# ckawoalt/Deep-Q-Learning_TRON

Hardware: AMD Instinct MI355X
Metric: env-steps/sec (higher is better)
Workload: dtype i8; 1 GPU; 65536 parallel 24x24 TRON envs per GPU, mode=none, random actions (in-kernel Philox), autoreset, obs=codes for both players; synthetic persistent rollout (no consumer reads the intermediate observations); envs_per_gpu=65536, grid=24x24, parallelism=env-shard x1

## Files before the change

### deep-q-learning_tron_amd/csrc/tron_env.hip

```cpp
#include "tron_device.hpp"
#include "tron_minimax.hpp"
#include "../../include/tron_hip.h"

#include <hip/hip_runtime.h>
#include <stdint.h>
#include <stdio.h>
#include <stdlib.h>
#include <math.h>
#include <string.h>
#include <new>
#include <type_traits>
#include <type_traits>

using namespace tron;

namespace {

constexpr int WAVE = 64;
constexpr int BLOCK = 256;
constexpr int DK = 6;

struct StepOut {
    int8_t *done;
    int8_t *winner;
// ... 801 lines not shown
    tally = 0u;
}

template <bool TAPE>
__device__ __forceinline__ void roll_helper(const Params &P, int env, bool autoreset, const uint4 &st, const uint4 &rs, int k_steps,
                                            int lane, uint2 *aring, uint32_t *sring, const uint32_t *cring, const StepOut &out,
                                            int wave, int gw, bool mine, const int8_t *tape, uint32_t game_starts, uint32_t *hand, bool handed)
{
    ROLL_HSTAMP(0);
    const uint32_t seed = P.seed, stream = P.stream;
    const int W = P.W, fair = P.fair, S = P.S;
    const uint32_t tick0 = st.w - ((autoreset && (st.y & META_DONE)) ? 1u : 0u), ep0 = rs.y;
    const int nb = (k_steps + ROLL_R - 1) / ROLL_R;
    uint32_t *abytes = reinterpret_cast<uint32_t *>(aring);
    uint32_t hi = 0u;
    uint32_t *const hme = hand + (mine ? (size_t)env : 0u);
    const size_t hn = (size_t)P.N;
    bool have_actions = false;
    if (handed) {
        uint32_t hw[ROLL_HAND_DWORDS];
#pragma unroll
        for (int i = 0; i < ROLL_HAND_DWORDS; ++i) hw[i] = 0u;
        hw[ROLL_HAND_DWORDS - 1] = ep0 + 2u * (uint32_t)ROLL_R;
        if (mine) {
            const uint32_t *q = hme;
#pragma unroll
            for (int i = 0; i < ROLL_HAND_DWORDS; ++i, q += hn) hw[i] = *q;
        }
#pragma unroll
        for (int i = 0; i < 2 * ROLL_R; ++i) sring[i * WAVE + lane] = hw[i];
        hi = hw[ROLL_HAND_DWORDS - 1] - ep0;
        if constexpr (!TAPE) {
            have_actions = __all(hw[2 * ROLL_R + 1] != ROLL_HAND_NO_ACTIONS) != 0;
            if (have_actions) aring[lane] = make_uint2(hw[2 * ROLL_R], hw[2 * ROLL_R + 1]);
        }
    }
    for (int b = -1; b < nb; ++b) {
        uint32_t base = 0u;
        if (b > 0) {
            ROLL_HSTAMP_BLOCK(b, 0);
            __syncthreads();
            ROLL_HSTAMP_BLOCK(b, 1);
        }
        const bool last = b + 1 >= nb;
        if (last && !autoreset) break;
        if (b >= 0) base = (b ? cring[(b & 1) * WAVE + lane] : 0u) + (uint32_t)ROLL_R;
        const uint32_t to = base + (uint32_t)min(ROLL_R, k_steps - (last ? b : b + 1) * ROLL_R);
        if (last) {
            if constexpr (!TAPE) {
#pragma nounroll
                for (int d = 0; d < ROLL_R / 4; ++d) {
                    uint32_t v = 0u;
#pragma unroll
                    for (uint32_t i = 0; i < 4u; ++i) {
                        uint32_t x[4];
                        philox4x32_10((uint32_t)env, tick0 + (uint32_t)k_steps + (uint32_t)(d * 4) + i, RNG_STEP, 0u, seed, stream, x);
                        v |= action_byte(x[0], x[1]) << (8u * i);
                    }
                    if (mine) hme[(size_t)(2 * ROLL_R + d) * hn] = v;
                }
            } else if (mine) {
                hme[(size_t)(2 * ROLL_R + 1) * hn] = ROLL_HAND_NO_ACTIONS;
            }
        } else if (TAPE || !(b < 0 && have_actions)) {
            if constexpr (!TAPE) {
#pragma nounroll
                for (int d = 0; d < ROLL_R / 4; ++d) {
                    const uint32_t s0 = (uint32_t)((b + 1) * ROLL_R + d * 4);
                    uint32_t v = 0u;
#pragma unroll
                    for (uint32_t i = 0; i < 4u; ++i) {
                        uint32_t x[4];
                        philox4x32_10((uint32_t)env, tick0 + s0 + i, RNG_STEP, 0u, seed, stream, x);
                        v |= action_byte(x[0], x[1]) << (8u * i);
                    }
                    abytes[(((s0 / ROLL_R) & 1u) * WAVE + (uint32_t)lane) * (ROLL_R / 4) + ((s0 / 4u) & (ROLL_R / 4 - 1))] = v;
                }
            } else {
                const int s0 = (b + 1) * ROLL_R;
                const uint16_t *row = reinterpret_cast<const uint16_t *>(tape) + (size_t)s0 * (size_t)P.N + (size_t)env;
                uint32_t t[ROLL_R];
#pragma unroll
                for (int i = 0; i < ROLL_R; ++i) t[i] = (mine && s0 + i < k_steps) ? row[(size_t)i * (size_t)P.N] : 0u;
                uint32_t v[2] = {0u, 0u};
#pragma unroll
                for (int i = 0; i < ROLL_R; ++i) v[i >> 2] |= ((t[i] & 3u) | ((t[i] >> 6) & 0xCu)) << (8 * (i & 3));
                aring[((b + 1) & 1) * WAVE + lane] = make_uint2(v[0], v[1]);
            }
        }
        if (autoreset) {
            const uint32_t upto = b < 0 ? to - min(game_starts, to) : to;
#pragma nounroll
            for (uint32_t j = hi + 1u; j <= upto; ++j)
                sring[((ep0 + j) & (2u * ROLL_R - 1u)) * WAVE + (uint32_t)lane] = start_cells_word(S, make_game_starts(seed, stream, W, fair, (uint32_t)env, ep0 + j));
            hi = max(hi, to);
        }
        if (last) {
            if (mine) {
                uint32_t hw[2 * ROLL_R];
#pragma unroll
                for (int i = 0; i < 2 * ROLL_R; ++i) hw[i] = sring[i * WAVE + lane];
                uint32_t *q = hme;
#pragma unroll
                for (int i = 0; i < 2 * ROLL_R; ++i, q += hn) *q = hw[i];
                q[2u * hn] = ep0 + hi;
            }
            ROLL_HSTAMP(ROLL_HSTAMPS - 2);
            break;
        }
        if (b < 0) {
            ROLL_HSTAMP(1);
            ROLL_HSTAMP(2);
            __syncthreads();
            ROLL_HSTAMP(3);
        }
    }
}

__device__ __forceinline__ int roll_cell(int S, int r, int c) { return __mul24(r + 1, S) + (c + 1); }
typedef __attribute__((address_space(3))) uint32_t lds_u32;
__device__ __forceinline__ uint32_t lds_cell_dword(uint32_t board_lds, uint32_t cell) { return board_lds + (cell >> 3) * 4u; }
__device__ __forceinline__ uint32_t lds_cell_shift(uint32_t cell) { return (cell & 7u) * 4u; }
__device__ __forceinline__ void lds_set_nibble(uint32_t dword_lds, uint32_t shift, uint32_t nib)
{
    asm volatile("ds_mskor_b32 %0, %1, %2" : : "v"(dword_lds), "v"(0xFu << shift), "v"(nib << shift) : "memory");
}

template <bool TAPE, bool REC = false>
__device__ __forceinline__ void roll_resident(kernarg_t *kp, int E, int epw, uint32_t cpe, uint32_t flags, const StepOut &out,
                                              int k_steps, unsigned char *smem, const int8_t *tape, unsigned long long *emask, uint32_t *hand)
{
    const uint32_t sd = 2u * cpe + 1u;
    uint32_t *boards = reinterpret_cast<uint32_t *>(smem);
    uint32_t *tmpl = boards + (size_t)E * sd;

    const int tid = threadIdx.x;
    const int lane = tid & 63;
    const int gw = (int)(blockDim.x >> 7);
    const int hw_wave = __builtin_amdgcn_readfirstlane(tid >> 6);
    const bool helper = hw_wave >= gw;
    const int wave = helper ? hw_wave - gw : hw_wave;
    uint16_t *wlist = reinterpret_cast<uint16_t *>(tmpl + 2u * cpe + (size_t)wave * (32u * cpe));
    uint32_t *rings = tmpl + ((2u * cpe + (size_t)gw * (32u * cpe) + 1u) & ~(size_t)1u) + (size_t)wave * ROLL_RING_DWORDS;
    uint2 *aring = reinterpret_cast<uint2 *>(rings);
    uint32_t *sring = rings + 4 * WAVE;
    uint32_t *cring = sring + 2 * ROLL_R * WAVE;
    const bool autoreset = (flags & TRON_STEP_AUTORESET) != 0u, nonrev = !TAPE && (flags & TRON_STEP_NONREVERSING) != 0u;
    const int we0 = wave * epw;
    const int e0 = (int)blockIdx.x * E + we0;
    const int env = e0 + lane;
    uint32_t *wboards = boards + (size_t)we0 * sd;
    uint32_t *board = wboards + (size_t)lane * sd;
    unsigned char *cellb = reinterpret_cast<unsigned char *>(board);
    bool mine;
    int8_t *oenv;
    uint4 st = make_uint4(0u, 0u, 0u, 0u), rs = make_uint4(0u, 0u, 0u, 0u);
    uint2 ab = make_uint2(0u, 0u);
    unsigned long long mask = 0ull;
    unsigned long long dirty = 0ull;
    unsigned long long stale = 0ull;
    bool st_dirty = false;
    uint32_t nres = 0u;
    uint32_t n_steps = 0u, n_w1 = 0u, n_w2 = 0u, n_draw = 0u;
    uint32_t tally = 0u;
    int S = 0;

    ROLL_STAMP_LAUNCH(0);
    {
        Params P;
        load_params_scalar(P, kp);
        const int G = P.G;
        S = P.S;
        const int ne = min(min(epw, E - we0), P.N - e0);
        mine = lane < ne;
        oenv = P.obs_state + (size_t)(mine ? env : 0) * 2u * G;
        const bool masked = (flags & ROLL_ENTRY_MASKED) != 0u;
        const bool handed = (flags & ROLL_ENTRY_HANDED) != 0u;
        const uint32_t game_starts = masked && autoreset && !handed ? (uint32_t)min(ROLL_GAME_STARTS, min(ROLL_R, k_steps)) : 0u;
        if (mine) {
            st = P.st4[env];
            if (autoreset) rs = P.rs4[env];
            if (masked && !helper) mask = emask[env];
        }
        for (uint32_t d = (uint32_t)tid; d < 2u * cpe; d += blockDim.x) {
            const uint32_t *fw = reinterpret_cast<const uint32_t *>(P.fresh);
            const uint32_t last = (uint32_t)G / 4u - 1u;
            const uint32_t f[2] = {fw[min(2u * d, last)], fw[min(2u * d + 1u, last)]};
            uint32_t v = 0u;
#pragma unroll
            for (uint32_t j = 0; j < 8u; ++j)
                if (d * 8u + j < (uint32_t)G)
                    v |= ((int8_t)(f[j >> 2] >> (8u * (j & 3u))) == TRON_EMPTY ? NIB_EMPTY : NIB_WALL) << (4u * j);
            tmpl[d] = v;
        }
        __syncthreads();
        if (helper) {
            roll_helper<TAPE>(P, env, autoreset, st, rs, k_steps, lane, aring, sring, cring, out, wave, gw, mine, tape, game_starts, hand, handed);
            return;
        }
        if (masked) {
            stale = ~mask & (cpe >= 64u ? ~0ull : (1ull << cpe) - 1ull);
            unsigned long long m = mask;
            const uint32_t cnt = (uint32_t)__popcll(m);
            uint32_t pos = 0u, T = 0u;
#pragma unroll
            for (uint32_t b = 0; b < 7u; ++b) {
                const unsigned long long bm = __ballot(((cnt >> b) & 1u) != 0u);
                pos += __builtin_amdgcn_mbcnt_hi((uint32_t)(bm >> 32), __builtin_amdgcn_mbcnt_lo((uint32_t)bm, 0u)) << b;
                T += (uint32_t)__popcll(bm) << b;
            }
            if (T) {
                for (uint32_t p = pos; m; ++p) {
                    wlist[p] = (uint16_t)(((uint32_t)lane << 6) | ((uint32_t)__ffsll((long long)m) - 1u));
                    m &= m - 1ull;
                }
                __builtin_amdgcn_fence(__ATOMIC_ACQ_REL, "wavefront");
                __builtin_amdgcn_wave_barrier();
                const int8_t *const obase = P.obs_state + (size_t)e0 * 2u * G;
                constexpr uint32_t GF = 8u;
                for (uint32_t t0 = 0u; t0 < T; t0 += 64u * GF) {
                    uint32_t ent[GF];
                    uint4 v[GF];
#pragma unroll
                    for (uint32_t j = 0; j < GF; ++j) ent[j] = wlist[min(t0 + 64u * j + (uint32_t)lane, T - 1u)];
#pragma unroll
                    for (uint32_t j = 0; j < GF; ++j)
                        if (t0 + 64u * j < T)
                            v[j] = load_chunk<true>(obase + (__umul24(ent[j] >> 6, 2u * (uint32_t)G) + (ent[j] & 63u) * 16u));
#pragma unroll
                    for (uint32_t j = 0; j < GF; ++j)
                        if (t0 + 64u * j < T && t0 + 64u * j + (uint32_t)lane < T) {
                            const uint32_t own = ent[j] >> 6, k = ent[j] & 63u;
                            const int nb = G - (int)k * 16;
                            if (nb <= 4) v[j].y = 0u;
                            if (nb <= 8) v[j].z = 0u;
                            if (nb <= 12) v[j].w = 0u;
                            uint32_t *b = wboards + __umul24(own, sd) + 2u * k;
                            b[0] = pack_codes8(v[j].x, v[j].y);
                            b[1] = pack_codes8(v[j].z, v[j].w);
                        }
                }
                __builtin_amdgcn_fence(__ATOMIC_ACQ_REL, "wavefront");
                __builtin_amdgcn_wave_barrier();
            }
            if (game_starts) {
                const uint32_t to = (uint32_t)min(ROLL_R, k_steps);
#pragma nounroll
                for (uint32_t j = to - game_starts + 1u; j <= to; ++j)
                    sring[((rs.y + j) & (2u * ROLL_R - 1u)) * WAVE + (uint32_t)lane] = start_cells_word(S, make_game_starts(P.seed, P.stream, P.W, P.fair, (uint32_t)env, rs.y + j));
            }
        } else {
            const bool ck = (uint32_t)lane < cpe;
            const int nb = G - lane * 16;
            const uint32_t t0 = ck ? tmpl[2 * lane] : 0u, t1 = ck ? tmpl[2 * lane + 1] : 0u;
            constexpr int PF = 8;
            for (int e = 0; e < ne; e += PF) {
                uint4 v[PF];
#pragma unroll
                for (int j = 0; j < PF; ++j)
                    v[j] = load_chunk<true>(P.obs_state + (size_t)(e0 + min(e + j, ne - 1)) * 2u * G + (ck ? lane * 16 : 0));
#pragma unroll
                for (int j = 0; j < PF; ++j) {
                    if (e + j >= ne) break;
                    uint32_t p0 = 0u, p1 = 0u;
                    if (ck) {
                        if (nb <= 4) v[j].y = 0u;
                        if (nb <= 8) v[j].z = 0u;
                        if (nb <= 12) v[j].w = 0u;
                        p0 = pack_codes8(v[j].x, v[j].y);
                        p1 = pack_codes8(v[j].z, v[j].w);
                        uint32_t *b = wboards + (size_t)(e + j) * sd + 2 * lane;
                        b[0] = p0;
                        b[1] = p1;
                    }
                    const unsigned long long diff = __ballot(ck && (p0 != t0 || p1 != t1));
                    if (lane == e + j) mask = diff;
                }
            }
        }
        ROLL_HSTAMP(ROLL_HSTAMPS - 1);
        __syncthreads();
    }
    const unsigned long long mask0 = mask;
    size_t row = 0;

    int cell[2];
    {
        int r[2], c[2];
        unpack_pos(st.x, r, c);
        cell[0] = roll_cell(S, r[0], c[0]);
        cell[1] = roll_cell(S, r[1], c[1]);
    }
    const uint32_t deltas = cell_deltas(S);
    uint32_t alive = st.y & 3u;
    bool done = (st.y & META_DONE) != 0u;
    int winner = (int)((st.y >> 4) & 3u);
    uint32_t last[2] = {(st.y >> 8) & 0xFu, (st.y >> 12) & 0xFu};
    if (mine && !done) dirty = (1ull << (cell[0] >> 4)) | (1ull << (cell[1] >> 4));
    uint32_t eplen = st.z, tick = st.w;
    rs.z = start_cells_word(S, rs.z);
    const uint32_t board_lds = (uint32_t)(uintptr_t)(lds_u32 *)board;
    uint32_t hdw[2] = {lds_cell_dword(board_lds, (uint32_t)cell[0]), lds_cell_dword(board_lds, (uint32_t)cell[1])};
    uint32_t hsh[2] = {lds_cell_shift((uint32_t)cell[0]), lds_cell_shift((uint32_t)cell[1])};

    for (int s0 = 0; s0 < k_steps; s0 += ROLL_R) {
        if (s0) {
            if (out.totals && (s0 & 127) == 0) roll_flush_tally(tally, n_steps, n_w1, n_w2, n_draw);
            cring[((s0 / ROLL_R) & 1) * WAVE + lane] = nres;
            __syncthreads();
        }
        ab = aring[((s0 / ROLL_R) & 1) * WAVE + lane];
        asm volatile("" : "+v"(ab.x), "+v"(ab.y));
        const int s1 = min(s0 + ROLL_R, k_steps);
        auto block_steps = [&](auto nr) __attribute__((always_inline)) {
        constexpr bool NONREV = decltype(nr)::value;
#pragma nounroll
        for (int s = s0; s < s1; ++s) {
            Params P;
            if constexpr (REC) load_params_scalar(P, kp);
            ROLL_STAMP(0);

            const bool stepped = mine && !done;
            float rw0 = 0.0f, rw1 = 0.0f;
            if (stepped) {
                const uint32_t abyte = ab.x & 0xFFu;
                const int a[2] = {draw_action_byte(abyte, 0, last[0], NONREV), draw_action_byte(abyte, 1, last[1], NONREV)};
                int ncell[2];
                unsigned long long nbit[2];
                uint32_t nk[2], ndw[2], nsh[2];
#pragma unroll
                for (int p = 0; p < 2; ++p) {
                    ncell[p] = cell[p] + cell_delta(deltas, a[p]);
                    nk[p] = (uint32_t)ncell[p] >> 4;
                    asm("" : "+v"(nk[p]));
                    nbit[p] = 1ull << nk[p];
                    ndw[p] = lds_cell_dword(board_lds, (uint32_t)ncell[p]);
                    nsh[p] = lds_cell_shift((uint32_t)ncell[p]);
                }
                uint32_t bw[2], tc0[2], tc1[2];
                bool sl[2];
#pragma unroll
                for (int p = 0; p < 2; ++p) {
                    bw[p] = *(lds_u32 *)(uintptr_t)ndw[p];
                    tc0[p] = tmpl[2u * nk[p]];
                    tc1[p] = tmpl[2u * nk[p] + 1u];
                    sl[p] = (stale & nbit[p]) != 0ull;
                }
                uint32_t tf[2];
#pragma unroll
                for (int p = 0; p < 2; ++p) {
                    const uint32_t tw = (ncell[p] & 8) ? tc1[p] : tc0[p];
                    tf[p] = ((sl[p] ? tw : bw[p]) >> nsh[p]) & 15u;
                }
                plain_targets(cell, ncell, tf, NIB_P1_BODY, NIB_P2_BODY, NIB_P1_HEAD);
#pragma unroll
                for (int p = 0; p < 2; ++p) alive = collide(alive, p, tf[p] == NIB_EMPTY);
                done = settle(alive, ncell, winner);
                if constexpr (REC)
                    if (out.reward) step_rewards(P, done, winner, eplen, rw0, rw1);
                last[0] = (uint32_t)a[0] + 1u;
                last[1] = (uint32_t)a[1] + 1u;
                eplen += 1u;
                tick += 1u;
                st_dirty = true;
                if (!(done && autoreset)) {
#pragma unroll
                    for (int p = 0; p < 2; ++p) {
                        if (sl[p]) {
                            board[2u * nk[p]] = tc0[p];
                            board[2u * nk[p] + 1u] = tc1[p];
                            stale &= ~nbit[p];
                        }
                    }
                    lds_set_nibble(hdw[0], hsh[0], NIB_P1_BODY);
                    lds_set_nibble(hdw[1], hsh[1], NIB_P2_BODY);
                    lds_set_nibble(ndw[0], nsh[0], NIB_P1_HEAD);
                    lds_set_nibble(ndw[1], nsh[1], NIB_P2_HEAD);
                    const unsigned long long nb = nbit[0] | nbit[1];
                    mask |= nb;
                    dirty |= nb;
                }
#pragma unroll
                for (int p = 0; p < 2; ++p) {
                    cell[p] = ncell[p];
                    hdw[p] = ndw[p];
                    hsh[p] = nsh[p];
                }
            }
            const bool fin = done;
            const int win = winner;
            ROLL_STAMP(1);

            if (mine && done && autoreset) {
                alive = META_ALIVE0 | META_ALIVE1;
                done = false;
                winner = 0;
                last[0] = last[1] = 0u;
                eplen = 0u;
                st_dirty = true;
                cell[0] = (int)(rs.z & 0xFFFFu);
                cell[1] = (int)(rs.z >> 16);
#pragma unroll
                for (int p = 0; p < 2; ++p) {
                    hdw[p] = lds_cell_dword(board_lds, (uint32_t)cell[p]);
                    hsh[p] = lds_cell_shift((uint32_t)cell[p]);
                }
                const uint32_t k1 = (uint32_t)cell[0] >> 4, k2 = (uint32_t)cell[1] >> 4;
                const unsigned long long heads = (1ull << k1) | (1ull << k2);
                dirty |= mask | heads;
                stale = (stale | mask) & ~heads;
                mask = heads;
                const uint32_t ta[2] = {tmpl[2u * k1], tmpl[2u * k1 + 1u]}, tb[2] = {tmpl[2u * k2], tmpl[2u * k2 + 1u]};
                board[2u * k1] = ta[0];
                board[2u * k1 + 1u] = ta[1];
                board[2u * k2] = tb[0];
                board[2u * k2 + 1u] = tb[1];
                lds_set_nibble(hdw[0], hsh[0], NIB_P1_HEAD);
                lds_set_nibble(hdw[1], hsh[1], NIB_P2_HEAD);
                rs.y += 1u;
                nres += 1u;
                rs.z = sring[(rs.y & (2u * ROLL_R - 1u)) * WAVE + lane];
            }
            ROLL_STAMP(2);

            if constexpr (REC) {
                const uint32_t n = (uint32_t)P.N;
                if (mine) {
                    if (out.done) (out.done + row)[(uint32_t)env] = (int8_t)fin;
                    if (out.winner) (out.winner + row)[(uint32_t)env] = (int8_t)win;
                    if (out.reward) (reinterpret_cast<float2 *>(out.reward) + row)[(uint32_t)env] = make_float2(rw0, rw1);
                }
                row += n;
            }
            if (out.totals && stepped) tally += 1u + (fin ? 1u << ((0x00100818u >> (8 * win)) & 31u) : 0u);
            ab.x = (ab.x >> 8) | (ab.y << 24);
            ab.y >>= 8;
            ROLL_STAMP(3);
        }
        };
        if (nonrev) block_steps(std::true_type{});
        else block_steps(std::false_type{});
    }

    ROLL_STAMP_LAUNCH(1);
    {
        Params P;
        load_params_scalar(P, kp);
        const int G = P.G;
        dirty &= mask | mask0;
        const uint32_t tail = (uint32_t)G & 15u;
        if (tail && ((dirty >> (cpe - 1u)) & 1ull)) {
            dirty &= ~(1ull << (cpe - 1u));
            const uint32_t k = cpe - 1u, cb = k * 16u;
            const uint32_t *const src = ((stale >> k) & 1ull) ? tmpl : board;
            const uint32_t p0 = src[2u * k], p1 = src[2u * k + 1u];
            uint32_t w1[4], w2[4];
            expand_codes8(p0, w1[0], w1[1]);
            expand_codes8(p1, w1[2], w1[3]);
            expand_codes8(swap_nibbles8(p0), w2[0], w2[1]);
            expand_codes8(swap_nibbles8(p1), w2[2], w2[3]);
            uint32_t *q1 = reinterpret_cast<uint32_t *>(oenv + cb), *q2 = reinterpret_cast<uint32_t *>(oenv + G + cb);
            q1[0] = w1[0];
            q2[0] = w2[0];
            if (tail > 4u) {
                q1[1] = w1[1];
                q2[1] = w2[1];
            }
            if (tail > 8u) {
                q1[2] = w1[2];
                q2[2] = w2[2];
            }
        }
        const uint32_t cnt = (uint32_t)__popcll(dirty);
        uint32_t pos = 0u, T = 0u;
#pragma unroll
        for (uint32_t b = 0; b < 7u; ++b) {
            const unsigned long long m = __ballot(((cnt >> b) & 1u) != 0u);
            pos += __builtin_amdgcn_mbcnt_hi((uint32_t)(m >> 32), __builtin_amdgcn_mbcnt_lo((uint32_t)m, 0u)) << b;
            T += (uint32_t)__popcll(m) << b;
        }
        if (T) {
            for (uint32_t p = pos; dirty; ++p) {
                const uint32_t k = (uint32_t)__ffsll((long long)dirty) - 1u;
                wlist[p] = (uint16_t)(((uint32_t)(stale >> k) & 1u) << 12 | ((uint32_t)lane << 6) | k);
                dirty &= dirty - 1ull;
            }
            __builtin_amdgcn_fence(__ATOMIC_ACQ_REL, "wavefront");
            __builtin_amdgcn_wave_barrier();
            int8_t *const obase = P.obs_state + (size_t)e0 * 2u * G;
            uint32_t idx = (uint32_t)lane;
            uint32_t ent = wlist[min(idx, T - 1u)];
            while (idx < T) {
                const uint32_t own = (ent >> 6) & 63u, k = ent & 63u;
                const uint32_t *const ob = ((ent >> 12) ? tmpl : wboards + __umul24(own, sd)) + 2u * k;
                const uint32_t p0 = ob[0], p1 = ob[1];
                idx += 64u;
                ent = wlist[min(idx, T - 1u)];
                uint32_t w1[4], w2[4];
                expand_codes8(p0, w1[0], w1[1]);
                expand_codes8(p1, w1[2], w1[3]);
                expand_codes8(swap_nibbles8(p0), w2[0], w2[1]);
                expand_codes8(swap_nibbles8(p1), w2[2], w2[3]);
                int8_t *const q = obase + (__umul24(own, 2u * (uint32_t)G) + k * 16u);
                *reinterpret_cast<U4A4 *>(q) = U4A4{w1[0], w1[1], w1[2], w1[3]};
                *reinterpret_cast<U4A4 *>(q + G) = U4A4{w2[0], w2[1], w2[2], w2[3]};
            }
        }
        ROLL_STAMP_LAUNCH(2);
        if (mine && st_dirty) {
            P.st4[env] = make_uint4(cells_pos(S, cell[0], cell[1]), pack_meta(alive, done, winner, (int)last[0] - 1, (int)last[1] - 1), eplen, tick);
        }
        if (mine) emask[env] = mask;
        if (mine && nres) {
            uint32_t envp = rs.w;
#pragma nounroll
            for (uint32_t back = min(nres, 2u) - 1u; (int)back >= 0; --back) {
                const NewGame ng = make_game(P.seed, P.stream, P.W, P.fair, (uint32_t)env, rs.y - back);
                if (back) envp = pack_envp(ng.w0, ng.w1, ng.degree);
                else rs.w = pack_envp(ng.w0, ng.w1, ng.degree);
            }
            rs.x = envp;
            rs.z = cells_pos(S, (int)(rs.z & 0xFFFFu), (int)(rs.z >> 16));
            P.rs4[env] = rs;
        }
    }
    ROLL_STAMP_LAUNCH(3);
#ifndef TRON_STAMPS
    if (out.totals) roll_flush_tally(tally, n_steps, n_w1, n_w2, n_draw);
    if (out.totals && lane == 0) {
        if (n_steps) atomicAdd(&out.totals[0], (unsigned long long)n_steps);
        if (n_w1) atomicAdd(&out.totals[1], (unsigned long long)n_w1);
        if (n_w2) atomicAdd(&out.totals[2], (unsigned long long)n_w2);
        if (n_draw) atomicAdd(&out.totals[3], (unsigned long long)n_draw);
    }
#endif
}

__global__ __launch_bounds__(2 * BLOCK) void k_obs_roll(Params P, int E, int epw, uint32_t cpe, uint32_t flags, StepOut out, int k_steps,
                                                        unsigned long long *__restrict__ emask, uint32_t *__restrict__ hand)
{
    extern __shared__ __attribute__((aligned(16))) unsigned char smem[];
    kernarg_t *kp = (kernarg_t *)__builtin_amdgcn_kernarg_segment_ptr();
    roll_resident<false>(kp, E, epw, cpe, flags & ~TRON_ROLLOUT_RESIDENT, out, k_steps, smem, nullptr, emask, hand);
}

__global__ __launch_bounds__(2 * BLOCK) void k_obs_roll_tape(Params P, int E, int epw, uint32_t cpe, uint32_t flags, StepOut out, int k_steps,
                                                             const int8_t *__restrict__ tape, unsigned long long *__restrict__ emask, uint32_t *__restrict__ hand)
{
    extern __shared__ __attribute__((aligned(16))) unsigned char smem[];
    kernarg_t *kp = (kernarg_t *)__builtin_amdgcn_kernarg_segment_ptr();
    roll_resident<true>(kp, E, epw, cpe, flags, out, k_steps, smem, tape, emask, hand);
}

__global__ __launch_bounds__(2 * BLOCK) void k_obs_roll_tape_rec(Params P, int E, int epw, uint32_t cpe, uint32_t flags, StepOut out, int k_steps,
                                                                 const int8_t *__restrict__ tape, unsigned long long *__restrict__ emask, uint32_t *__restrict__ hand)
{
    extern __shared__ __attribute__((aligned(16))) unsigned char smem[];
    kernarg_t *kp = (kernarg_t *)__builtin_amdgcn_kernarg_segment_ptr();
    roll_resident<true, true>(kp, E, epw, cpe, flags, out, k_steps, smem, tape, emask, hand);
}

__global__ __launch_bounds__(BLOCK) void k_obs_roll_walk(Params P, int E, uint32_t cpe, uint32_t cpe_magic, uint32_t flags,
                                                        StepOut out, int k_steps, int ntiles)
{
    extern __shared__ __attribute__((aligned(16))) unsigned char smem[];
    __shared__ unsigned long long acc[4];
    StepOut lo = out;
    if (out.totals) {
        if (threadIdx.x < 4) acc[threadIdx.x] = 0ull;
        lo.totals = acc;
        __syncthreads();
    }
    flags &= ~TRON_ROLLOUT_RESIDENT;
    kernarg_t *kp = (kernarg_t *)__builtin_amdgcn_kernarg_segment_ptr();
    for (int s = 0; s < k_steps; ++s)
        for (int t = (int)blockIdx.x; t < ntiles; t += (int)gridDim.x) {
            kernarg_t *q = kp;
            asm volatile("" : "+s"(q));
            Params Pl;
            load_params(Pl, q);
            obs_tile<true>(Pl, E, cpe, cpe_magic, nullptr, flags, lo, t, smem);
            __syncthreads();
        }
    if (out.totals && threadIdx.x < 4 && acc[threadIdx.x]) atomicAdd(&out.totals[threadIdx.x], acc[threadIdx.x]);
}

template <class F> struct first_kernel_arg;
template <class R, class A0, class... A> struct first_kernel_arg<R (*)(A0, A...)> { typedef A0 type; };
static_assert(std::is_same<first_kernel_arg<decltype(&k_obs_roll)>::type, Params>::value,
              "k_obs_roll re-reads Params from kernarg offset 0: Params must stay its first parameter");
static_assert(std::is_same<first_kernel_arg<decltype(&k_obs_roll_walk)>::type, Params>::value, "k_obs_roll_walk re-reads Params from kernarg offset 0");
static_assert(std::is_same<first_kernel_arg<decltype(&k_obs_roll_tape)>::type, Params>::value, "k_obs_roll_tape re-reads Params from kernarg offset 0");
static_assert(std::is_same<first_kernel_arg<decltype(&k_obs_roll_tape_rec)>::type, Params>::value, "k_obs_roll_tape_rec re-reads Params from kernarg offset 0");
static_assert(std::is_trivially_copyable<Params>::value && alignof(Params) <= 8 && sizeof(Params) % 4 == 0,
              "Params is block-copied from the kernel-argument segment with scalar loads");

#ifndef TRON_SLIDE_KERNARG_REREAD
#define TRON_SLIDE_KERNARG_REREAD 1
#endif
__global__ __launch_bounds__(BLOCK) void k_obs_roll_slide(Params P, int E, uint32_t cpe, uint32_t cpe_magic, uint32_t flags,
                                                         StepOut out, int k_steps, int ntiles)
{
    extern __shared__ __attribute__((aligned(16))) unsigned char smem[];
    __shared__ unsigned long long acc[4];
    StepOut lo = out;
    if (out.totals) {
        if (threadIdx.x < 4) acc[threadIdx.x] = 0ull;
        lo.totals = acc;
        __syncthreads();
    }
    const bool resident = (flags & TRON_ROLLOUT_RESIDENT) != 0u && (int)gridDim.x == ntiles;
    flags &= ~TRON_ROLLOUT_RESIDENT;
#if TRON_SLIDE_KERNARG_REREAD
    kernarg_t *kp = (kernarg_t *)__builtin_amdgcn_kernarg_segment_ptr();
#endif
    for (int s = 0; s < k_steps; ++s)
        for (int t = (int)blockIdx.x; t < ntiles; t += (int)gridDim.x) {
#if TRON_SLIDE_KERNARG_REREAD
            kernarg_t *q = kp;
            asm volatile("" : "+s"(q));
            Params Pl;
            load_params(Pl, q);
            obs_tile<true, true>(Pl, E, cpe, cpe_magic, nullptr, flags, lo, t, smem, resident && s > 0, resident);
#else
            obs_tile<true, true>(P, E, cpe, cpe_magic, nullptr, flags, lo, t, smem, resident && s > 0, resident);
#endif
            __syncthreads();
        }
    if (out.totals && threadIdx.x < 4 && acc[threadIdx.x]) atomicAdd(&out.totals[threadIdx.x], acc[threadIdx.x]);
}
static_assert(std::is_same<first_kernel_arg<decltype(&k_obs_roll_slide)>::type, Params>::value, "k_obs_roll_slide may re-read Params from kernarg offset 0");

template <int DUMMY>
__global__ __launch_bounds__(BLOCK) void k_inc(Params P, uint32_t cpe, const int8_t *__restrict__ actions,
                                               uint32_t flags, StepOut out)
{
    __shared__ uint4 tmpl[640];
    __shared__ uint4 rec_rs[WAVE];
    __shared__ uint32_t rec_nstart[WAVE];
    __shared__ uint32_t rec_heads[WAVE];
    const int G = P.G, S = P.S, W = P.W;
    const int tid = threadIdx.x, lane = tid & 63, wave = tid >> 6;
    const int env = blockIdx.x * WAVE + lane;
    const bool mine = env < P.N;
    const bool autoreset = (flags & TRON_STEP_AUTORESET) != 0u, nonrev = (flags & TRON_STEP_NONREVERSING) != 0u;

    uint4 st = make_uint4(0u, META_DONE, 0u, 0u), rs = make_uint4(0u, 0u, 0u, 0u);
    uint32_t act = 0u;
    if (mine && wave == 0) {
        st = P.st4[env];
        if (actions) act = reinterpret_cast<const uint16_t *>(actions)[env];
    }
    if (mine && wave == 1 && autoreset) rs = P.rs4[env];
    if (autoreset)
        for (uint32_t d = (uint32_t)tid; d < cpe * 16u; d += BLOCK)
            reinterpret_cast<int8_t *>(tmpl)[d] = (d < (uint32_t)G) ? (P.fresh[d] == TRON_EMPTY ? (int8_t)1 : (int8_t)-1) : (int8_t)0;
    if (wave == 1 && autoreset) {
        rec_nstart[lane] = rs.z;
        if (mine) {
            const NewGame ng = make_game(P.seed, P.stream, W, P.fair, (uint32_t)env, rs.y + 1u);
            rec_rs[lane] = make_uint4(rs.w, rs.y + 1u, pack_pos(ng.r1, ng.c1, ng.r2, ng.c2), pack_envp(ng.w0, ng.w1, ng.degree));
        }
    }

    bool restart = false, done = false, stepped = false;
    int winner = 0;
    uint4 new_st = st;
    if (wave == 0) {
        int8_t *o1 = P.obs_state + (size_t)(mine ? env : 0) * 2u * G, *o2 = o1 + G;
        typedef CodeCells C;
        uint32_t m = st.y;
        int r[2], c[2];
        unpack_pos(st.x, r, c);
        done = (m & META_DONE) != 0;
        stepped = mine && !done;
        winner = (int)((m >> 4) & 3u);
        float rw0 = 0.0f, rw1 = 0.0f;
        if (stepped) {
            int a[2];
            if (!actions) {
                uint32_t x[4];
                philox4x32_10((uint32_t)env, st.w, RNG_STEP, 0u, P.seed, P.stream, x);
                a[0] = draw_action(x[0], (m >> 8) & 0xFu, nonrev);
                a[1] = draw_action(x[1], (m >> 12) & 0xFu, nonrev);
            } else {
                a[0] = (int)(act & 3u);
                a[1] = (int)((act >> 8) & 3u);
            }
            int old[2], f[2], tf[2];
#pragma unroll
            for (int p = 0; p < 2; ++p) {
                int dr, dc;
                action_delta(a[p], dr, dc);
                old[p] = cell_index(S, r[p], c[p]);
                r[p] += dr;
                c[p] += dc;
                f[p] = cell_index(S, r[p], c[p]);
            }
            tf[0] = o1[f[0]];
            tf[1] = o1[f[1]];
            plain_targets(old, f, tf, (int)C::P1_BODY, (int)C::P2_BODY, (int)C::P1_HEAD);
            uint32_t alive = m & 3u;
#pragma unroll
            for (int p = 0; p < 2; ++p) alive = collide(alive, p, W, r[p], c[p], tf[p] == C::EMPTY);
            done = settle(alive, r, c, winner);
            step_rewards(P, done, winner, st.z, rw0, rw1);
            new_st = stepped_st4(r, c, pack_meta(alive, done, winner, a[0], a[1]), st.z, st.w);
            if (!(done && autoreset)) {
                o1[old[0]] = C::P1_BODY; o2[old[0]] = C::P2_BODY;
                o1[old[1]] = C::P2_BODY; o2[old[1]] = C::P1_BODY;
                o1[f[0]] = C::P1_HEAD;   o2[f[0]] = C::P2_HEAD;
                o1[f[1]] = C::P2_HEAD;   o2[f[1]] = C::P1_HEAD;
                P.st4[env] = new_st;
            }
        }
        if (mine) {
            if (out.done) out.done[env] = (int8_t)done;
            if (out.winner) out.winner[env] = (int8_t)winner;
            if (out.reward) reinterpret_cast<float2 *>(out.reward)[env] = make_float2(rw0, rw1);
        }
        if (out.totals) {
            const int wn = (stepped && done) ? winner : -1;
            const unsigned long long bs = __ballot(stepped);
            const unsigned long long b1 = __ballot(wn == 1), b2 = __ballot(wn == 2), b0 = __ballot(wn == 0);
// ... 961 lines not shown
```

Before: 85.30 billion env-steps/s.

## Merge autoreset board writes into step write path and prefetch reset state

Restructures the per-step rollout loop so the autoreset path and the normal step share one LDS write block, choosing the target cell, template words and refresh flags with selects instead of running two separate divergent blocks. The reset start cell's template words and the next start-cell ring entry are loaded speculatively every step, before the step logic, so their LDS latency overlaps with the step computation rather than sitting on the reset path. The stale-bit test now uses a shift instead of a 64-bit mask. This trades extra unconditional LDS loads and select instructions per step for less divergence and shorter dependency chains on reset.

```diff
diff --git a/deep-q-learning_tron_amd/csrc/tron_env.hip b/deep-q-learning_tron_amd/csrc/tron_env.hip
--- a/deep-q-learning_tron_amd/csrc/tron_env.hip
+++ b/deep-q-learning_tron_amd/csrc/tron_env.hip
@@ -1127,6 +1127,7 @@
     const uint32_t board_lds = (uint32_t)(uintptr_t)(lds_u32 *)board;
     uint32_t hdw[2] = {lds_cell_dword(board_lds, (uint32_t)cell[0]), lds_cell_dword(board_lds, (uint32_t)cell[1])};
     uint32_t hsh[2] = {lds_cell_shift((uint32_t)cell[0]), lds_cell_shift((uint32_t)cell[1])};
+    uint32_t snext = (rs.y + 1u) & (2u * ROLL_R - 1u);
 
     for (int s0 = 0; s0 < k_steps; s0 += ROLL_R) {
         if (s0) {
@@ -1146,30 +1147,37 @@
             ROLL_STAMP(0);
 
             const bool stepped = mine && !done;
+            const uint32_t scell_a = rs.z & 0xFFFFu, scell_b = rs.z >> 16;
+            uint32_t sk_a = scell_a >> 4, sk_b = scell_b >> 4;
+            asm("" : "+v"(sk_a), "+v"(sk_b));
+            const uint32_t ts0_a = tmpl[2u * sk_a], ts1_a = tmpl[2u * sk_a + 1u], ts0_b = tmpl[2u * sk_b], ts1_b = tmpl[2u * sk_b + 1u];
+            const uint32_t nx = sring[snext * WAVE + (uint32_t)lane];
             float rw0 = 0.0f, rw1 = 0.0f;
+            int ncell_a = 0, ncell_b = 0;
+            uint32_t nk_a = 0u, nk_b = 0u, tc0_a = 0u, tc0_b = 0u, tc1_a = 0u, tc1_b = 0u;
+            bool sl_a = false, sl_b = false;
             if (stepped) {
+                int ncell[2];
+                uint32_t nk[2], tc0[2], tc1[2];
+                bool sl[2];
                 const uint32_t abyte = ab.x & 0xFFu;
                 const int a[2] = {draw_action_byte(abyte, 0, last[0], NONREV), draw_action_byte(abyte, 1, last[1], NONREV)};
-                int ncell[2];
-                unsigned long long nbit[2];
-                uint32_t nk[2], ndw[2], nsh[2];
+                uint32_t ndw[2], nsh[2];
 #pragma unroll
                 for (int p = 0; p < 2; ++p) {
                     ncell[p] = cell[p] + cell_delta(deltas, a[p]);
                     nk[p] = (uint32_t)ncell[p] >> 4;
                     asm("" : "+v"(nk[p]));
-                    nbit[p] = 1ull << nk[p];
                     ndw[p] = lds_cell_dword(board_lds, (uint32_t)ncell[p]);
                     nsh[p] = lds_cell_shift((uint32_t)ncell[p]);
                 }
-                uint32_t bw[2], tc0[2], tc1[2];
-                bool sl[2];
+                uint32_t bw[2];
 #pragma unroll
                 for (int p = 0; p < 2; ++p) {
                     bw[p] = *(lds_u32 *)(uintptr_t)ndw[p];
                     tc0[p] = tmpl[2u * nk[p]];
                     tc1[p] = tmpl[2u * nk[p] + 1u];
-                    sl[p] = (stale & nbit[p]) != 0ull;
+                    sl[p] = ((stale >> nk[p]) & 1ull) != 0ull;
                 }
                 uint32_t tf[2];
 #pragma unroll
@@ -1188,63 +1196,67 @@
                 eplen += 1u;
                 tick += 1u;
                 st_dirty = true;
-                if (!(done && autoreset)) {
-#pragma unroll
-                    for (int p = 0; p < 2; ++p) {
-                        if (sl[p]) {
-                            board[2u * nk[p]] = tc0[p];
-                            board[2u * nk[p] + 1u] = tc1[p];
-                            stale &= ~nbit[p];
-                        }
+                ncell_a = ncell[0], ncell_b = ncell[1];
+                nk_a = nk[0], nk_b = nk[1];
+                tc0_a = tc0[0], tc0_b = tc0[1], tc1_a = tc1[0], tc1_b = tc1[1];
+                sl_a = sl[0], sl_b = sl[1];
+            }
+            asm volatile("" : : "v"(ts0_a), "v"(ts1_a), "v"(ts0_b), "v"(ts1_b), "v"(nx));
+            const bool fin = done;
+            const int win = winner;
+            const bool restart = mine && done && autoreset;
+            ROLL_STAMP(1);
+            if (stepped || restart) {
+                if (restart) {
+                    dirty |= mask;
+                    stale |= mask;
+                    mask = 0ull;
+                }
+                const int wcell[2] = {restart ? (int)scell_a : ncell_a, restart ? (int)scell_b : ncell_b};
+                uint32_t wk[2] = {restart ? sk_a : nk_a, restart ? sk_b : nk_b};
+                const uint32_t wd0[2] = {restart ? ts0_a : tc0_a, restart ? ts0_b : tc0_b}, wd1[2] = {restart ? ts1_a : tc1_a, restart ? ts1_b : tc1_b};
+                const bool rf[2] = {restart || sl_a, restart || sl_b};
+                uint32_t wdw[2], wsh[2];
+                unsigned long long nb = 0ull;
+#pragma unroll
+                for (int p = 0; p < 2; ++p) {
+                    asm("" : "+v"(wk[p]));
+                    wdw[p] = lds_cell_dword(board_lds, (uint32_t)wcell[p]);
+                    wsh[p] = lds_cell_shift((uint32_t)wcell[p]);
+                    const unsigned long long wbit = 1ull << wk[p];
+                    nb |= wbit;
+                    if (rf[p]) {
+                        board[2u * wk[p]] = wd0[p];
+                        board[2u * wk[p] + 1u] = wd1[p];
+                        stale &= ~wbit;
                     }
+                }
+                if (!restart) {
                     lds_set_nibble(hdw[0], hsh[0], NIB_P1_BODY);
                     lds_set_nibble(hdw[1], hsh[1], NIB_P2_BODY);
-                    lds_set_nibble(ndw[0], nsh[0], NIB_P1_HEAD);
-                    lds_set_nibble(ndw[1], nsh[1], NIB_P2_HEAD);
-                    const unsigned long long nb = nbit[0] | nbit[1];
-                    mask |= nb;
-                    dirty |= nb;
                 }
+                lds_set_nibble(wdw[0], wsh[0], NIB_P1_HEAD);
+                lds_set_nibble(wdw[1], wsh[1], NIB_P2_HEAD);
+                mask |= nb;
+                dirty |= nb;
 #pragma unroll
                 for (int p = 0; p < 2; ++p) {
-                    cell[p] = ncell[p];
-                    hdw[p] = ndw[p];
-                    hsh[p] = nsh[p];
+                    cell[p] = wcell[p];
+                    hdw[p] = wdw[p];
+                    hsh[p] = wsh[p];
                 }
             }
-            const bool fin = done;
-            const int win = winner;
-            ROLL_STAMP(1);
-
-            if (mine && done && autoreset) {
+            if (restart) {
                 alive = META_ALIVE0 | META_ALIVE1;
                 done = false;
                 winner = 0;
                 last[0] = last[1] = 0u;
                 eplen = 0u;
                 st_dirty = true;
-                cell[0] = (int)(rs.z & 0xFFFFu);
-                cell[1] = (int)(rs.z >> 16);
-#pragma unroll
-                for (int p = 0; p < 2; ++p) {
-                    hdw[p] = lds_cell_dword(board_lds, (uint32_t)cell[p]);
-                    hsh[p] = lds_cell_shift((uint32_t)cell[p]);
-                }
-                const uint32_t k1 = (uint32_t)cell[0] >> 4, k2 = (uint32_t)cell[1] >> 4;
-                const unsigned long long heads = (1ull << k1) | (1ull << k2);
-                dirty |= mask | heads;
-                stale = (stale | mask) & ~heads;
-                mask = heads;
-                const uint32_t ta[2] = {tmpl[2u * k1], tmpl[2u * k1 + 1u]}, tb[2] = {tmpl[2u * k2], tmpl[2u * k2 + 1u]};
-                board[2u * k1] = ta[0];
-                board[2u * k1 + 1u] = ta[1];
-                board[2u * k2] = tb[0];
-                board[2u * k2 + 1u] = tb[1];
-                lds_set_nibble(hdw[0], hsh[0], NIB_P1_HEAD);
-                lds_set_nibble(hdw[1], hsh[1], NIB_P2_HEAD);
                 rs.y += 1u;
                 nres += 1u;
-                rs.z = sring[(rs.y & (2u * ROLL_R - 1u)) * WAVE + lane];
+                rs.z = nx;
+                snext = (snext + 1u) & (2u * ROLL_R - 1u);
             }
             ROLL_STAMP(2);
 
```

New measurement: 87.66 billion env-steps/s (median of 6 runs). 1.03x the previous value.
